# TimZaman/dotaclient

Hardware: NVIDIA H100
Metric: optimizer_steps_per_sec (higher is better)
Workload: dtype f32

## Files before the change

### dotaclient_b200/_lib.py

```python
import ctypes
import os

_HERE = os.path.dirname(os.path.abspath(__file__))
LIB_PATH = os.path.join(_HERE, "libdotaclient_b200.so")

_c = ctypes
_vp, _i32, _i64, _f32, _f64, _sz = _c.c_void_p, _c.c_int, _c.c_int64, _c.c_float, _c.c_double, _c.c_size_t
_ptr5 = _c.c_void_p * 5


class GatherDesc(_c.Structure):
    _fields_ = [("src", _vp), ("dst", _vp), ("outer", _i64), ("src_cols", _i64), ("row_bytes", _i64)]

SIGNATURES = {
    "dc_version": (_i32, []),
    "dc_last_error": (_c.c_char_p, []),
    "dc_device_info": (_i32, [_c.POINTER(_i32)] * 3),
    "dc_gae_scan": (_i32, [_vp, _i32, _vp, _vp, _i32, _vp, _vp, _f64, _f64, _vp, _vp, _vp]),
    "dc_vtrace_scan": (_i32, [_vp, _i32, _vp, _vp, _vp, _vp, _i32, _vp, _vp, _f64, _f64, _f64, _f64, _vp, _vp, _vp, _vp]),
    "dc_gae_scan_indexed": (_i32, [_vp, _i32, _vp, _i64, _vp, _vp, _i32, _vp, _vp, _f64, _f64, _vp, _vp, _vp]),
    "dc_vtrace_scan_indexed": (_i32, [_vp, _i32, _vp, _i64, _vp, _vp, _vp, _vp, _i32, _vp, _vp, _f64, _f64, _f64, _f64, _vp,
                                      _vp, _vp, _vp]),
    "dc_gather_columns": (_i32, [_c.POINTER(GatherDesc), _i32, _vp, _i64, _vp]),
    "dc_gather_columns_fill": (_i32, [_c.POINTER(GatherDesc), _i32, _vp, _i64, _vp]),
    "dc_refresh_states": (_i32, [_i32, _i32, _vp, _vp, _i64, _i64, _vp, _vp, _vp, _i64, _i64, _i64, _vp, _vp, _vp, _vp, _vp,
                                 _vp, _vp]),
    "dc_rnn_workspace_bytes": (_sz, [_i32, _i32, _i32]),
    "dc_rnn_seq_fwd": (_i32, [_i32, _vp, _vp, _vp, _vp, _vp, _i32, _i32, _i32, _vp, _vp]),
    "dc_rnn_seq_bwd": (_i32, [_i32, _vp, _vp, _vp, _vp, _vp, _vp, _vp, _vp, _vp, _i32, _i32, _i32, _vp, _vp]),
    "dc_rnn_seq_fwd_reset": (_i32, [_i32, _vp, _vp, _vp, _vp, _vp, _vp, _vp, _vp, _i32, _i32, _i32, _i32, _vp, _vp]),
    "dc_rnn_seq_bwd_reset": (_i32, [_i32, _vp, _vp, _vp, _vp, _vp, _vp, _vp, _vp, _vp, _vp, _vp, _i32, _i32, _i32, _i32, _vp,
                                    _vp]),
    "dc_gemm_tf32x3_supported": (_i32, [_i64, _i32, _i32]),
    "dc_gemm_tf32x3": (_i32, [_vp, _i32, _vp, _i32, _vp, _vp, _i32, _i64, _i32, _i32, _i32, _vp]),
    "dc_gemm_wgrad_workspace_bytes": (_sz, [_i32, _i32]),
    "dc_gemm_wgrad_tf32x3": (_i32, [_vp, _i32, _vp, _i32, _i64, _i32, _i32, _vp, _i32, _vp, _i32, _vp, _vp]),
    "dc_unit_basic_bwd_workspace_bytes": (_sz, []),
    "dc_env_fwd": (_i32, [_vp, _vp, _vp, _vp, _i32, _i64, _vp]),
    "dc_env_bwd_workspace_bytes": (_sz, []),
    "dc_env_bwd": (_i32, [_vp, _vp, _i32, _vp, _vp, _vp, _i64, _vp, _vp]),
    "dc_unit_wgrad_routed": (_i32, [_vp, _vp, _i32, _vp, _vp, _i64, _i32, _vp, _vp, _vp, _vp]),
    "dc_unit_dgrad_fused": (_i32, [_vp, _vp, _i32, _vp, _vp, _i32, _vp, _vp, _vp, _vp, _vp, _i64, _i32, _vp, _vp, _i32, _vp, _vp]),
    "dc_unit_dgrad_fused_mask": (_i32, [_vp, _vp, _i32, _vp, _vp, _i32, _vp, _vp, _vp, _vp, _vp, _vp, _i64, _i32, _vp, _vp, _i32, _vp,
                                        _vp]),
    "dc_gemm_unit_max": (_i32, [_vp, _vp, _vp, _vp, _vp, _i32, _vp, _i64, _i32, _vp]),
    "dc_unit_embed_fwd": (_i32, [_vp, _vp, _vp, _vp, _vp, _vp, _vp, _vp, _i32, _vp, _i64, _i32, _vp]),
    "dc_unit_embed_fwd_mask": (_i32, [_vp, _vp, _vp, _vp, _vp, _vp, _vp, _vp, _vp, _i32, _vp, _i64, _i32, _vp]),
    "dc_target_unit_q_fwd": (_i32, [_vp, _i32, _c.c_void_p * 6, _vp, _vp, _vp, _i64, _vp]),
    "dc_target_unit_q_bwd": (_i32, [_vp, _c.c_void_p * 6, _vp, _vp, _vp, _i32, _i64, _vp]),
    "dc_ppo_loss_fwd_bwd": (_i32, [_ptr5, _ptr5, _ptr5, _vp, _vp, _vp, _vp, _i64, _f32, _f32, _f32, _ptr5, _vp, _vp,
                                   _vp, _vp, _vp]),
    "dc_ppo_loss_fwd_bwd_strided": (_i32, [_ptr5, _c.c_int64 * 5, _ptr5, _ptr5, _vp, _vp, _vp, _vp, _i64, _i64, _f32, _f32, _f32,
                                           _ptr5, _c.c_int64 * 5, _vp, _i64, _vp, _vp, _vp, _vp]),
    "dc_ppo_loss_fwd_bwd_dev": (_i32, [_ptr5, _c.c_int64 * 5, _ptr5, _ptr5, _vp, _vp, _vp, _vp, _i64, _vp, _i64, _vp,
                                       _ptr5, _c.c_int64 * 5, _vp, _i64, _vp, _vp, _vp, _vp, _vp]),
    "dc_ppo_loss_fwd_bwd_masked": (_i32, [_ptr5, _c.c_int64 * 5, _ptr5, _ptr5, _vp, _vp, _vp, _vp, _i64, _vp, _vp, _i64,
                                          _vp, _ptr5, _c.c_int64 * 5, _vp, _i64, _vp, _vp, _vp, _vp, _vp]),
    "dc_ppo_loss_fwd_bwd_joint": (_i32, [_ptr5, _c.c_int64 * 5, _ptr5, _ptr5, _vp, _vp, _vp, _vp, _i64, _vp, _vp, _i64,
                                         _vp, _ptr5, _c.c_int64 * 5, _vp, _i64, _vp, _vp, _vp, _vp, _vp]),
    "dc_ppo_loss_fwd_bwd_kl": (_i32, [_ptr5, _c.c_int64 * 5, _ptr5, _ptr5, _vp, _vp, _vp, _vp, _vp, _i64, _vp, _vp, _i64,
                                      _vp, _i32, _ptr5, _c.c_int64 * 5, _vp, _i64, _vp, _vp, _vp, _vp, _vp, _vp]),
    "dc_selected_logp_rows": (_i32, [_ptr5, _ptr5, _ptr5, _i64, _vp, _vp, _vp]),
    "dc_value_norm_stats": (_i32, [_vp, _vp, _i64, _vp, _vp]),
    "dc_value_denorm": (_i32, [_vp, _i64, _i64, _f64, _f64, _vp, _vp]),
    "dc_value_head_rescale": (_i32, [_vp, _i64, _vp, _f64, _f64, _f64, _f64, _vp]),
    "dc_selected_logp": (_i32, [_ptr5, _ptr5, _ptr5, _i64, _vp, _vp]),
    "dc_select_actions": (_i32, [_ptr5, _c.c_int64 * 5, _ptr5, _vp, _i64, _vp, _vp, _vp]),
    "dc_grad_flags": (_i32, [_vp, _i64, _vp, _i32, _vp, _vp]),
    "dc_grad_finish": (_i32, [_vp, _vp, _vp, _vp, _vp, _vp, _vp, _vp, _i32, _i64, _f64, _f64, _f64, _f64, _f64, _vp, _vp,
                              _vp, _vp]),
    "dc_grad_finish_dev": (_i32, [_vp, _vp, _vp, _vp, _vp, _vp, _vp, _vp, _i32, _i64, _vp, _f64, _f64, _f64, _vp, _vp, _vp,
                                  _vp]),
    "dc_grad_finish_kl": (_i32, [_vp, _vp, _vp, _vp, _vp, _vp, _vp, _vp, _i32, _i64, _vp, _f64, _f64, _f64, _vp, _vp, _vp,
                                 _vp]),
}

PPO_WORKSPACE_BYTES = 512
FINISH_WORKSPACE_BYTES = 1024
LOSS_SLOTS = 16
HPARAM_SLOTS = 10
HP_LR, HP_E_CLIP, HP_ENTROPY_COEF, HP_VF_COEF, HP_MAX_GRAD_NORM, HP_VALUE_CLIP = range(6)
HP_VALUE_NORM_MEAN, HP_VALUE_NORM_STD = 6, 7
HP_KL_COEF, HP_KL_STOP = 8, 9
PPO_STATS_SLOTS = 24
STAT_APPROX_KL, STAT_CLIP_FRACTION, STAT_EXPLAINED_VAR = 0, 6, 12
STAT_JOINT_APPROX_KL, STAT_JOINT_CLIP_FRACTION = 13, 14
STAT_KL, STAT_KL_PENALTY = 16, 22
KL_ROW_FLOATS = 65
FINISH_KL_METRICS = 6
VTRACE_STATS_SLOTS = 8
GATHER_MAX_TENSORS = 32
REFRESH_MAX_LAYERS = 16
MAX_PARAM_TENSORS = 96

_lib = None


class NativeLibraryError(RuntimeError):
    pass


def load():
    global _lib
    if _lib is not None:
        return _lib
    if not os.path.exists(LIB_PATH):
        raise NativeLibraryError(
            "%s not found: build it with `python -m dotaclient_b200.build` (needs nvcc, sm_90a). "
            "dotaclient_b200 has no CPU fallback." % LIB_PATH)
    lib = ctypes.CDLL(LIB_PATH)
    for name, (res, args) in SIGNATURES.items():
        try:
            fn = getattr(lib, name)
        except AttributeError:
            continue
        fn.restype = res
        fn.argtypes = args
    _lib = lib
    return lib


def exported(name):
    lib = load()
    return hasattr(lib, name)


def check(rc, what):
    if rc != 0:
        msg = load().dc_last_error()
        raise RuntimeError("%s failed (code %d): %s" % (what, rc, msg.decode() if msg else "?"))


def ptr(t):
    return None if t is None else t.data_ptr()


def ptr5(tensors):
    return _ptr5(*[t.data_ptr() if t is not None else None for t in tensors])


def stream_ptr():
    import torch
    return torch.cuda.current_stream().cuda_stream
```

### dotaclient_b200/csrc/gemm_tf32x3.cu

```cuda
#include "dc_common.cuh"
#include "unit_basic.cuh"

namespace {

constexpr int BM = 128, BN = 128, BK = 32;
constexpr int kStages = 2;
constexpr int kTileBytes = BM * BK * 4;
constexpr int kStageBytes = 4 * kTileBytes;
constexpr int kProducerThreads = 128;
constexpr int kProducerGroups = kStages;
constexpr int kConsumerWarp0 = 4 * kProducerGroups;
constexpr int kConsumerThreads = 256;
constexpr int kThreads = kConsumerWarp0 * 32 + kConsumerThreads;
constexpr int kLdS = BN + 8;
constexpr int kDIn = kUnitFeatures;
constexpr size_t kOffStaging = (size_t)kStages * kStageBytes;
constexpr size_t kOffBars = kOffStaging + (size_t)BM * kLdS * 4;
constexpr size_t kSmemBytes = kOffBars + 128 + 1024 ;

#define DC_ACC8(b) "+f"(d[b]), "+f"(d[b + 1]), "+f"(d[b + 2]), "+f"(d[b + 3]), "+f"(d[b + 4]), "+f"(d[b + 5]), "+f"(d[b + 6]), "+f"(d[b + 7])
__device__ __forceinline__ void wgmma_m64n128k8(float (&d)[64], uint64_t desc_a, uint64_t desc_b) {
    asm volatile(
        "{\n\t.reg .pred p;\n\tsetp.ne.b32 p, %66, 0;\n\t"
        "wgmma.mma_async.sync.aligned.m64n128k8.f32.tf32.tf32 "
// ... 872 lines not shown
            const int s = j % kWgStages;
            dc_mbar_wait(&empty[s], ((j / kWgStages) & 1) ^ 1);
            unsigned char *st = ring + (size_t)s * kWgStageBytes;
            const uint32_t xs = dc_smem_u32(st + 2 * kTileBytes);
#pragma unroll
            for (int r = 0; r < BK / 4; ++r) {
                const int row = (t >> 5) + 4 * r;
                const bool ok = xc_in && t0 + row < tend;
                cp_async16(xs + (row * kWgLdX + 4 * xc) * 4, X + (ok ? (size_t)(t0 + row) * ldx + n0 + 4 * xc : 0), ok ? 16u : 0u);
            }
            cp_async_arrive(&full[s]);
            store_row_k(va, st, st + kTileBytes, t);
            asm volatile("fence.proxy.async.shared::cta;" ::: "memory");
            __syncwarp();
            if (lane == 0) dc_mbar_arrive(&full[s]);
        }
        colsum_s[g * 128 + t] = cs;
        asm volatile("cp.async.wait_all;" ::: "memory");
    } else {
        const int ct = threadIdx.x - kConsumerWarp0 * 32, wg = ct >> 7, w4 = (ct >> 5) & 3, q = lane & 3;
        const int rlo = 64 * wg + 16 * w4 + (lane >> 2);
        float d[64];
#pragma unroll
        for (int i = 0; i < 64; ++i) d[i] = 0.f;
        uint32_t ahi[2][4] = {}, alo[2][4] = {};
#pragma unroll
        for (int i = 0; i < 64; ++i) dc_reg_fence(d[i]);
        float *pt = part_w + ((size_t)split * tiles_mn + tile) * BM * BN + ct * 4;
        const auto flush = [&](bool add) {
            dc_wgmma_wait0();
#pragma unroll
            for (int k = 0; k < 64; ++k) dc_reg_fence(d[k]);
            if (add) {
#pragma unroll
                for (int m = 0; m < 16; ++m)
                    asm volatile("red.global.add.v4.f32 [%0], {%1, %2, %3, %4};" ::"l"(pt + m * kConsumerThreads * 4), "f"(d[4 * m]),
                                 "f"(d[4 * m + 1]), "f"(d[4 * m + 2]), "f"(d[4 * m + 3]) : "memory");
            } else {
#pragma unroll
                for (int m = 0; m < 16; ++m)
                    *reinterpret_cast<float4 *>(pt + m * kConsumerThreads * 4) = make_float4(d[4 * m], d[4 * m + 1], d[4 * m + 2], d[4 * m + 3]);
            }
#pragma unroll
            for (int k = 0; k < 64; ++k) d[k] = 0.f;
#pragma unroll
            for (int k = 0; k < 64; ++k) dc_reg_fence(d[k]);
        };
        int j = 0;
        do {
            const int j_end = min(my_chunks, j + kWgFlush);
            for (; j < j_end; ++j) {
                const int s = j % kWgStages;
                dc_mbar_wait(&full[s], (j / kWgStages) & 1);
                const uint32_t st = dc_smem_u32(ring + (size_t)s * kWgStageBytes);
                const uint32_t xk = st + 2 * kTileBytes + (q * kWgLdX + rlo) * 4;
                float v[16];
#pragma unroll
                for (int ks = 0; ks < BK / 8; ++ks) {
                    const uint32_t x8 = xk + 8 * ks * kWgLdX * 4;
                    v[4 * ks] = lds_f32(x8);
                    v[4 * ks + 1] = lds_f32(x8 + 8 * 4);
                    v[4 * ks + 2] = lds_f32(x8 + 4 * kWgLdX * 4);
                    v[4 * ks + 3] = lds_f32(x8 + (4 * kWgLdX + 8) * 4);
                }
                const uint64_t b_hi = dc_wgmma_desc(st), b_lo = dc_wgmma_desc(st + kTileBytes);
#pragma unroll
                for (int ks = 0; ks < BK / 8; ++ks) {
                    const int b = ks & 1;
#pragma unroll
                    for (int e = 0; e < 4; ++e) {
                        const float h = dc_tf32_rna(v[4 * ks + e]);
                        ahi[b][e] = __float_as_uint(h);
                        alo[b][e] = __float_as_uint(v[4 * ks + e] - h);
                    }
                    dc_wgmma_fence();
                    const uint64_t adv = (uint64_t)(ks * 2);
                    wgmma_m64n128k8_rs(d, ahi[b][0], ahi[b][1], ahi[b][2], ahi[b][3], b_lo + adv);
                    wgmma_m64n128k8_rs(d, alo[b][0], alo[b][1], alo[b][2], alo[b][3], b_hi + adv);
                    wgmma_m64n128k8_rs(d, ahi[b][0], ahi[b][1], ahi[b][2], ahi[b][3], b_hi + adv);
                    dc_wgmma_commit();
                    wgmma_wait1();
#pragma unroll
                    for (int e = 0; e < 4; ++e) asm volatile("" : "+r"(ahi[b ^ 1][e]), "+r"(alo[b ^ 1][e])::"memory");
                    if (ks == 0 && j > 0) {
                        __syncwarp();
                        if (lane == 0) dc_mbar_arrive(&empty[(j - 1) % kWgStages]);
                    }
                }
            }
            flush(j > kWgFlush);
        } while (j < my_chunks);
    }
    __syncthreads();
    if (part_b != nullptr && n0 == 0 && threadIdx.x < 128 && m0 + (int)threadIdx.x < No)
        part_b[(size_t)split * No + m0 + threadIdx.x] = colsum_s[threadIdx.x] + colsum_s[128 + threadIdx.x];
}

constexpr int kRedRows = 8;
__global__ void __launch_bounds__(32 * kRedRows) wgrad_reduce_kernel(const float *__restrict__ part_w, const float *__restrict__ part_b,
                                                                     int nsplit, int No, int Ni, float *__restrict__ dW, int ldw,
                                                                     float *__restrict__ db, int accumulate) {
    __shared__ float4 sh[kRedRows][32];
    const int x = threadIdx.x & 31, y = threadIdx.x >> 5;
    const int n_blocks = (Ni + BN - 1) / BN, tiles_mn = ((No + BM - 1) / BM) * n_blocks;
    const int total4 = tiles_mn * (BM * BN / 4), bias4 = db != nullptr ? No / 4 : 0;
    const int idx = blockIdx.x * 32 + x;
    const float *src = nullptr;
    size_t stride = 0;
    if (idx < total4) {
        src = part_w + (size_t)idx * 4;
        stride = (size_t)tiles_mn * BM * BN;
    } else if (idx < total4 + bias4) {
        src = part_b + (size_t)(idx - total4) * 4;
        stride = (size_t)No;
    }
    float4 acc = make_float4(0.f, 0.f, 0.f, 0.f);
    if (src != nullptr) {
#pragma unroll 4
        for (int s = y; s < nsplit; s += kRedRows) {
            const float4 v = __ldg(reinterpret_cast<const float4 *>(src + (size_t)s * stride));
            acc.x += v.x; acc.y += v.y; acc.z += v.z; acc.w += v.w;
        }
    }
    sh[y][x] = acc;
    __syncthreads();
    if (y == 0 && src != nullptr) {
        if (idx < total4) {
            const int tile = idx / (BM * BN / 4), r = idx % (BM * BN / 4), m = r / kConsumerThreads, ct = r % kConsumerThreads;
            const int o = (tile / n_blocks) * BM + 8 * m + 2 * (ct & 3);
            const int i = (tile % n_blocks) * BN + 64 * (ct >> 7) + 16 * ((ct >> 5) & 3) + ((ct & 31) >> 2);
            float *p[4];
            float v[4];
#pragma unroll
            for (int e = 0; e < 4; ++e) {
                const int oe = o + (e & 1), ie = i + 8 * (e >> 1);
                p[e] = oe < No && ie < Ni ? dW + (size_t)oe * ldw + ie : nullptr;
                v[e] = accumulate && p[e] != nullptr ? *p[e] : 0.f;
            }
#pragma unroll
            for (int r = 0; r < kRedRows; ++r) { v[0] += sh[r][x].x; v[1] += sh[r][x].y; v[2] += sh[r][x].z; v[3] += sh[r][x].w; }
#pragma unroll
            for (int e = 0; e < 4; ++e)
                if (p[e] != nullptr) *p[e] = v[e];
        } else {
            float *dst = db + (size_t)(idx - total4) * 4;
            float4 t = accumulate ? *reinterpret_cast<const float4 *>(dst) : make_float4(0.f, 0.f, 0.f, 0.f);
#pragma unroll
            for (int r = 0; r < kRedRows; ++r) { t.x += sh[r][x].x; t.y += sh[r][x].y; t.z += sh[r][x].z; t.w += sh[r][x].w; }
            *reinterpret_cast<float4 *>(dst) = t;
        }
    }
}

}

extern "C" int dc_gemm_tf32x3_supported(int64_t M, int N, int K) { return M > 0 && N > 0 && K > 0 && N % 32 == 0 && K % BK == 0; }

template <int NU, bool kGenA = false>
static int launch_ws(const float *A, int lda, const float *B, int ldb, const float *bias, float *C, int ldc, int M, int N,
                     int K, int relu, float *C_copy, uint8_t *argmax, cudaStream_t st, GenA gen = GenA{}) {
    const int tile_rows = NU == 5 ? 60 : kWsRows;
    const int n_blocks = (N + BN - 1) / BN, m_blocks = (M + tile_rows - 1) / tile_rows;
    int per_block = dc_sm_count() / n_blocks;
    if (per_block < 1) per_block = 1;
    if (per_block > m_blocks) per_block = m_blocks;
    const size_t smem = kGenA ? kWsGenSmemBytes : kWsSmemBytes;
    DC_CUDA(cudaFuncSetAttribute(gemm_ws_kernel<NU, kGenA>, cudaFuncAttributeMaxDynamicSharedMemorySize, (int)smem));
    gemm_ws_kernel<NU, kGenA><<<n_blocks * per_block, kWsThreads, smem, st>>>(A, lda, B, ldb, bias, C, ldc, M, N, K, relu, C_copy,
                                                                             argmax, gen);
    DC_LAUNCH_OK();
    return DC_OK;
}

extern "C" int dc_gemm_tf32x3(const float *A, int lda, const float *B, int ldb, const float *bias, float *C, int ldc,
                              int64_t M, int N, int K, int relu, dc_stream_t stream) {
    DC_REQUIRE(A && B && C, DC_EINVAL, "dc_gemm_tf32x3: null pointer");
    DC_REQUIRE(dc_gemm_tf32x3_supported(M, N, K) && M < (1ll << 31) - BM, DC_EUNSUPPORTED,
               "dc_gemm_tf32x3: need N %% 32 == 0 and K %% 32 == 0 (M=%lld N=%d K=%d)", (long long)M, N, K);
    DC_REQUIRE(lda >= K && ldb >= K && ldc >= N && lda % 4 == 0 && ldb % 4 == 0 && ldc % 4 == 0, DC_EINVAL,
               "dc_gemm_tf32x3: leading dimensions must be >= extent and multiples of 4 floats");
    DC_REQUIRE(((uintptr_t)A & 15) == 0 && ((uintptr_t)B & 15) == 0 && ((uintptr_t)C & 15) == 0 && (!bias || ((uintptr_t)bias & 15) == 0),
               DC_EINVAL, "dc_gemm_tf32x3: pointers must be 16-byte aligned");
    if (K <= 4 * BK) return launch_ws<0>(A, lda, B, ldb, bias, C, ldc, (int)M, N, K, relu, nullptr, nullptr, dc_cu_stream(stream));
    const int tiles = (int)((M + BM - 1) / BM) * ((N + BN - 1) / BN);
    DC_CUDA(cudaFuncSetAttribute(gemm_tf32x3_kernel, cudaFuncAttributeMaxDynamicSharedMemorySize, (int)kSmemBytes));
    const int grid = tiles < dc_sm_count() ? tiles : dc_sm_count();
    gemm_tf32x3_kernel<<<grid, kThreads, kSmemBytes, dc_cu_stream(stream)>>>(A, lda, B, ldb, bias, C, ldc, (int)M, N, K, relu, 1, 0);
    DC_LAUNCH_OK();
    return DC_OK;
}

int dc_gemm_tf32x3_splitk(const float *A, int lda, const float *B, int ldb, float *part, int64_t M, int N, int K, int ksplit,
                          bool first_call, cudaStream_t st) {
    DC_REQUIRE(A && B && part && ksplit >= 1 && N % BN == 0 && K % (BK * ksplit) == 0 && M > 0, DC_EINVAL,
               "dc_gemm_tf32x3_splitk: bad arguments (M=%lld N=%d K=%d ksplit=%d)", (long long)M, N, K, ksplit);
    if (first_call)
        DC_CUDA(cudaFuncSetAttribute(gemm_tf32x3_kernel, cudaFuncAttributeMaxDynamicSharedMemorySize, (int)kSmemBytes));
    const int tiles = (int)((M + BM - 1) / BM) * (N / BN) * ksplit;
    const int grid = tiles < dc_sm_count() ? tiles : dc_sm_count();
    gemm_tf32x3_kernel<<<grid, kThreads, kSmemBytes, st>>>(A, lda, B, ldb, nullptr, part, N, (int)M, N, K, 0, ksplit, (long long)M * N);
    DC_LAUNCH_OK();
    return DC_OK;
}

static int wgrad_tiles(int No, int Ni) { return ((No + BM - 1) / BM) * ((Ni + BN - 1) / BN); }

static int wgrad_splits(int No, int Ni) {
    const int tiles_mn = wgrad_tiles(No, Ni);
    const int n = dc_sm_count() / tiles_mn;
    return n < 1 ? 1 : n;
}

extern "C" size_t dc_gemm_wgrad_workspace_bytes(int No, int Ni) {
    if (No <= 0 || Ni <= 0 || No % 32 || Ni % 32) return 0;
    const int nsplit = wgrad_splits(No, Ni);
    return ((size_t)nsplit * wgrad_tiles(No, Ni) * BM * BN + (size_t)nsplit * No) * sizeof(float);
}

extern "C" int dc_gemm_wgrad_tf32x3(const float *dY, int ldy, const float *X, int ldx, int64_t T, int No, int Ni, float *dW,
                                    int ldw, float *db, int accumulate, void *workspace, dc_stream_t stream) {
    DC_REQUIRE(dY && X && dW && workspace, DC_EINVAL, "dc_gemm_wgrad_tf32x3: null pointer");
    DC_REQUIRE(T > 0 && T < (1ll << 31) - BK && No > 0 && Ni > 0 && No % 32 == 0 && Ni % 32 == 0, DC_EUNSUPPORTED,
               "dc_gemm_wgrad_tf32x3: need No %% 32 == 0 and Ni %% 32 == 0 (T=%lld No=%d Ni=%d)", (long long)T, No, Ni);
    DC_REQUIRE(ldy >= No && ldx >= Ni && ldw >= Ni && ldy % 4 == 0 && ldx % 4 == 0 && ldw % 4 == 0, DC_EINVAL,
               "dc_gemm_wgrad_tf32x3: bad leading dimension");
    DC_REQUIRE(((uintptr_t)dY & 15) == 0 && ((uintptr_t)X & 15) == 0 && ((uintptr_t)dW & 15) == 0 && ((uintptr_t)workspace & 15) == 0 &&
                   ((uintptr_t)db & 15) == 0,
               DC_EINVAL, "dc_gemm_wgrad_tf32x3: pointers must be 16-byte aligned");
    const int tiles_mn = wgrad_tiles(No, Ni), nsplit = wgrad_splits(No, Ni);
    float *part_w = reinterpret_cast<float *>(workspace);
    float *part_b = db ? part_w + (size_t)nsplit * tiles_mn * BM * BN : nullptr;
    cudaStream_t st = dc_cu_stream(stream);
    DC_CUDA(cudaFuncSetAttribute(gemm_wgrad_kernel<0>, cudaFuncAttributeMaxDynamicSharedMemorySize, (int)kWgSmemBytes));
    gemm_wgrad_kernel<0><<<tiles_mn * nsplit, kThreads, kWgSmemBytes, st>>>(dY, ldy, nullptr, nullptr, X, ldx, (int)T, No, Ni,
                                                                                      nsplit, part_w, part_b);
    DC_LAUNCH_OK();
    const int total4 = tiles_mn * (BM * BN / 4) + (db ? No / 4 : 0);
    wgrad_reduce_kernel<<<(total4 + 31) / 32, 32 * kRedRows, 0, st>>>(part_w, part_b, nsplit, No, Ni, dW, ldw, db, accumulate);
    DC_LAUNCH_OK();
    return DC_OK;
}

extern "C" int dc_gemm_unit_max(const float *basic, const float *w, const float *bias, float *xmax, float *xmax_copy, int ld_x,
                                uint8_t *argmax, int64_t n_tokens, int n_units, dc_stream_t stream) {
    DC_REQUIRE(basic && w && bias && xmax && argmax && n_tokens > 0, DC_EINVAL, "dc_gemm_unit_max: null pointer / empty input");
    DC_REQUIRE(n_units == 5 || n_units == 16, DC_EUNSUPPORTED, "dc_gemm_unit_max: n_units=%d (5 or 16; 1-unit groups are plain GEMMs)", n_units);
    DC_REQUIRE(ld_x >= BN && n_tokens * n_units < (1ll << 31) - BM, DC_EINVAL, "dc_gemm_unit_max: bad ld_x / size");
    DC_REQUIRE(((uintptr_t)basic & 15) == 0 && ((uintptr_t)w & 15) == 0, DC_EINVAL, "dc_gemm_unit_max: pointers must be 16-byte aligned");
    const int M = (int)(n_tokens * n_units);
    cudaStream_t st = dc_cu_stream(stream);
    if (n_units == 5) return launch_ws<5>(basic, BN, w, BN, bias, xmax, ld_x, M, BN, BN, 0, xmax_copy, argmax, st);
    return launch_ws<16>(basic, BN, w, BN, bias, xmax, ld_x, M, BN, BN, 0, xmax_copy, argmax, st);
}

extern "C" int dc_unit_embed_fwd_mask(const float *units, const float *w_b, const float *b_b, float *basic_out, uint32_t *mask_out,
                                      const float *w, const float *bias, float *xmax, float *xmax_copy, int ld_x, uint8_t *argmax,
                                      int64_t n_tokens, int n_units, dc_stream_t stream) {
    DC_REQUIRE(units && w_b && b_b && w && bias && xmax && n_tokens > 0, DC_EINVAL, "dc_unit_embed_fwd: null pointer / empty input");
    DC_REQUIRE(n_units == 1 || n_units == 5 || n_units == 16, DC_EUNSUPPORTED, "dc_unit_embed_fwd: n_units=%d (1, 5 or 16)", n_units);
    DC_REQUIRE(n_units == 1 ? (argmax == nullptr && xmax_copy == nullptr) : argmax != nullptr, DC_EINVAL,
               "dc_unit_embed_fwd: the arg-max (and the copy) go with the max-pool of n_units 5 and 16 only");
    DC_REQUIRE(ld_x >= BN && ld_x % 4 == 0 && n_tokens * n_units < (1ll << 31) - BM, DC_EINVAL, "dc_unit_embed_fwd: bad ld_x / size");
    DC_REQUIRE(((uintptr_t)units & 15) == 0 && ((uintptr_t)basic_out & 15) == 0 && ((uintptr_t)w & 15) == 0 && ((uintptr_t)bias & 15) == 0 &&
                   ((uintptr_t)xmax & 15) == 0 && ((uintptr_t)xmax_copy & 15) == 0 && ((uintptr_t)mask_out & 15) == 0,
               DC_EINVAL, "dc_unit_embed_fwd: units, basic_out, mask_out, w, bias, xmax, xmax_copy must be 16-byte aligned");
    const int M = (int)(n_tokens * n_units);
    const GenA gen{units, w_b, b_b, basic_out, mask_out};
    cudaStream_t st = dc_cu_stream(stream);
    if (n_units == 1) return launch_ws<0, true>(nullptr, BN, w, BN, bias, xmax, ld_x, M, BN, BN, 0, nullptr, nullptr, st, gen);
    if (n_units == 5) return launch_ws<5, true>(nullptr, BN, w, BN, bias, xmax, ld_x, M, BN, BN, 0, xmax_copy, argmax, st, gen);
    return launch_ws<16, true>(nullptr, BN, w, BN, bias, xmax, ld_x, M, BN, BN, 0, xmax_copy, argmax, st, gen);
}

extern "C" int dc_unit_embed_fwd(const float *units, const float *w_b, const float *b_b, float *basic_out, const float *w, const float *bias,
                                 float *xmax, float *xmax_copy, int ld_x, uint8_t *argmax, int64_t n_tokens, int n_units,
                                 dc_stream_t stream) {
    return dc_unit_embed_fwd_mask(units, w_b, b_b, basic_out, nullptr, w, bias, xmax, xmax_copy, ld_x, argmax, n_tokens, n_units, stream);
}

extern "C" int dc_unit_dgrad_fused_mask(const float *d_xmax, const float *d_xmax2, int ld_dx, const uint8_t *argmax, const float *dlogits,
                                        int ld_dl, const float *att, const float *w_t, const float *units, const uint32_t *mask,
                                        const float *w_b, const float *b_b, int64_t n_tokens, int n_units, float *dw_b, float *db_b,
                                        int accumulate, void *workspace, dc_stream_t stream) {
    DC_REQUIRE(w_t && units && w_b && b_b && dw_b && db_b && workspace && n_tokens > 0, DC_EINVAL, "dc_unit_dgrad_fused: null pointer / empty input");
    DC_REQUIRE(n_units == 1 || n_units == 5 || n_units == 16, DC_EUNSUPPORTED, "dc_unit_dgrad_fused: n_units=%d (1, 5 or 16)", n_units);
    DC_REQUIRE((d_xmax == nullptr && d_xmax2 == nullptr) || (d_xmax != nullptr && ld_dx >= BN && ld_dx % 4 == 0), DC_EINVAL,
               "dc_unit_dgrad_fused: bad d_xmax / ld_dx");
    DC_REQUIRE(d_xmax == nullptr || n_units == 1 || argmax != nullptr, DC_EINVAL, "dc_unit_dgrad_fused: routing needs the arg-max");
    DC_REQUIRE((dlogits == nullptr) == (att == nullptr) && (dlogits == nullptr || ld_dl >= n_units), DC_EINVAL,
               "dc_unit_dgrad_fused: dlogits and att come together");
    DC_REQUIRE(n_tokens * n_units < (1ll << 31) - BM, DC_EINVAL, "dc_unit_dgrad_fused: too many rows");
    DC_REQUIRE(((uintptr_t)d_xmax & 15) == 0 && ((uintptr_t)d_xmax2 & 15) == 0 && ((uintptr_t)argmax & 3) == 0 && ((uintptr_t)att & 15) == 0 &&
                   ((uintptr_t)w_t & 15) == 0 && ((uintptr_t)units & 15) == 0 && ((uintptr_t)mask & 15) == 0 && ((uintptr_t)workspace & 15) == 0,
               DC_EINVAL, "dc_unit_dgrad_fused: d_xmax, att, w_t, units, mask must be 16-byte aligned (arg-max 4-byte)");
    const int n_tok = (int)n_tokens;
    const int tile_rows = BM - BM % n_units;
    int grid = (int)((n_tokens * n_units + tile_rows - 1) / tile_rows);
    if (grid > dc_sm_count()) grid = dc_sm_count();
    float *partial = reinterpret_cast<float *>(workspace);
    cudaStream_t st = dc_cu_stream(stream);
#define DC_LAUNCH_DGRAD(NU, MASK)                                                                                                    \
    do {                                                                                                                              \
        DC_CUDA(cudaFuncSetAttribute(unit_dgrad_kernel<NU, MASK>, cudaFuncAttributeMaxDynamicSharedMemorySize, (int)kDgSmemBytes)); \
        unit_dgrad_kernel<NU, MASK><<<grid, kThreads, kDgSmemBytes, st>>>(d_xmax, d_xmax2, ld_dx, argmax, dlogits, ld_dl, att, w_t,  \
                                                                          units, mask, w_b, b_b, n_tok, partial);                     \
    } while (0)
    if (mask != nullptr) {
        if (n_units == 1) DC_LAUNCH_DGRAD(1, true);
        else if (n_units == 5) DC_LAUNCH_DGRAD(5, true);
        else DC_LAUNCH_DGRAD(16, true);
    } else {
        if (n_units == 1) DC_LAUNCH_DGRAD(1, false);
        else if (n_units == 5) DC_LAUNCH_DGRAD(5, false);
        else DC_LAUNCH_DGRAD(16, false);
    }
#undef DC_LAUNCH_DGRAD
    DC_LAUNCH_OK();
    return dc_unit_basic_reduce(partial, grid, dw_b, db_b, accumulate, st);
}

extern "C" int dc_unit_dgrad_fused(const float *d_xmax, const float *d_xmax2, int ld_dx, const uint8_t *argmax, const float *dlogits,
                                   int ld_dl, const float *att, const float *w_t, const float *units, const float *w_b,
                                   const float *b_b, int64_t n_tokens, int n_units, float *dw_b, float *db_b, int accumulate,
                                   void *workspace, dc_stream_t stream) {
    return dc_unit_dgrad_fused_mask(d_xmax, d_xmax2, ld_dx, argmax, dlogits, ld_dl, att, w_t, units, nullptr, w_b, b_b, n_tokens, n_units,
                                    dw_b, db_b, accumulate, workspace, stream);
}

extern "C" int dc_unit_wgrad_routed(const float *d_xmax, const float *d_xmax2, int ld_dx, const uint8_t *argmax, const float *basic,
                                    int64_t n_tokens, int n_units, float *dW, float *db, void *workspace, dc_stream_t stream) {
    DC_REQUIRE(d_xmax && argmax && basic && dW && db && workspace && n_tokens > 0, DC_EINVAL, "dc_unit_wgrad_routed: null pointer / empty input");
    DC_REQUIRE(n_units == 5 || n_units == 16, DC_EUNSUPPORTED, "dc_unit_wgrad_routed: n_units=%d (5 or 16; a 1-unit group is dc_gemm_wgrad_tf32x3)", n_units);
    DC_REQUIRE(ld_dx >= BM && n_tokens * n_units < (1ll << 31) - BK, DC_EINVAL, "dc_unit_wgrad_routed: bad ld_dx / size");
    DC_REQUIRE(((uintptr_t)basic & 15) == 0 && ((uintptr_t)dW & 15) == 0 && ((uintptr_t)db & 15) == 0 && ((uintptr_t)workspace & 15) == 0,
               DC_EINVAL, "dc_unit_wgrad_routed: pointers must be 16-byte aligned");
    const int No = BM, Ni = BN, nsplit = wgrad_splits(No, Ni);
// ... 19 lines not shown
```

### include/dotaclient_b200.h

```cpp
#ifndef DOTACLIENT_B200_H
#define DOTACLIENT_B200_H

#include <stddef.h>
#include <stdint.h>

#ifdef __cplusplus
extern "C" {
#endif

#define DC_OK 0
#define DC_EINVAL (-1)
#define DC_EUNSUPPORTED (-2)

#define DC_CELL_GRU 0
#define DC_CELL_LSTM 1

#define DC_NUM_HEADS 5
#define DC_LOSS_SLOTS 16

typedef void *dc_stream_t;

int dc_version(void);
const char *dc_last_error(void);
int dc_device_info(int *sm_count, int *cc_major, int *cc_minor);

int dc_gae_scan(const float *rewards, int n_sub, const float *values, const int64_t *seg_off,
                int n_seg, const float *boot_value, const float *boot_reward, double gamma,
                double lam, float *adv, float *ret, dc_stream_t stream);

#define DC_VTRACE_STATS_SLOTS 8
int dc_vtrace_scan(const float *rewards, int n_sub, const float *values, const float *logp_target,
                   const float *logp_behaviour, const int64_t *seg_off, int n_seg, const int64_t *valid_len,
                   const float *boot_value, double gamma, double lam, double rho_clip, double c_clip, float *pg_adv,
                   float *vs, double *seg_stats, dc_stream_t stream);

int dc_gae_scan_indexed(const float *rewards, int n_sub, const float *values, int64_t ld_values, const int64_t *tok,
                        const int64_t *seg_off, int n_seg, const float *boot_value, const float *boot_reward,
                        double gamma, double lam, float *adv, float *ret, dc_stream_t stream);
int dc_vtrace_scan_indexed(const float *rewards, int n_sub, const float *values, int64_t ld_values,
                           const float *logp_target, const float *logp_behaviour, const int64_t *tok,
                           const int64_t *seg_off, int n_seg, const int64_t *valid_len, const float *boot_value,
                           double gamma, double lam, double rho_clip, double c_clip, float *pg_adv, float *vs,
                           double *seg_stats, dc_stream_t stream);

typedef struct {
    const void *src;
    void *dst;
    int64_t outer;
    int64_t src_cols;
    int64_t row_bytes;
} dc_gather_desc;
#define DC_GATHER_MAX_TENSORS 32
int dc_gather_columns(const dc_gather_desc *descs, int n_desc, const int64_t *index, int64_t n_index,
                      dc_stream_t stream);
int dc_gather_columns_fill(const dc_gather_desc *descs, int n_desc, const int64_t *index, int64_t n_index,
                           dc_stream_t stream);

#define DC_REFRESH_MAX_LAYERS 16
int dc_refresh_states(int n_layers, int H, const float *const *h_bufs, const float *const *c_bufs, int64_t R, int64_t t0,
                      const int64_t *step, const int64_t *rollout, const int64_t *slot, int64_t n, int64_t B, int64_t K,
                      float *h0, float *c0, float *reset_h, float *reset_c, double *partial, double *acc,
                      dc_stream_t stream);

size_t dc_rnn_workspace_bytes(int cell, int B, int H);
int dc_rnn_seq_fwd(int cell, float *gates, const float *w_hh, const float *b_hh, float *ybuf,
                   float *cbuf, int B, int S, int H, void *workspace, dc_stream_t stream);
int dc_rnn_seq_bwd(int cell, float *gates, const float *w_hh, const float *ybuf, float *cbuf,
                   const float *dy, const float *dhn, const float *dcn, float *dh0, float *dc0,
                   int B, int S, int H, void *workspace, dc_stream_t stream);

int dc_rnn_seq_fwd_reset(int cell, float *gates, const float *w_hh, const float *b_hh, float *ybuf, float *cbuf,
                         const int32_t *reset_slot, const float *reset_prev, const float *reset_pre, int K,
                         int B, int S, int H, void *workspace, dc_stream_t stream);
int dc_rnn_seq_bwd_reset(int cell, float *gates, const float *w_hh, const float *ybuf, float *cbuf,
                         const float *dy, const float *dhn, const float *dcn, float *dh0, float *dc0,
                         const int32_t *reset_slot, const float *reset_prev, int K,
                         int B, int S, int H, void *workspace, dc_stream_t stream);

int dc_gemm_tf32x3_supported(int64_t M, int N, int K);
int dc_gemm_tf32x3(const float *A, int lda, const float *B, int ldb, const float *bias, float *C, int ldc,
                   int64_t M, int N, int K, int relu, dc_stream_t stream);

size_t dc_gemm_wgrad_workspace_bytes(int No, int Ni);
int dc_gemm_wgrad_tf32x3(const float *dY, int ldy, const float *X, int ldx, int64_t T, int No, int Ni,
                         float *dW, int ldw, float *db, int accumulate, void *workspace, dc_stream_t stream);

size_t dc_unit_basic_bwd_workspace_bytes(void);
int dc_env_fwd(const float *env, const float *w_e, const float *b_e, float *out, int ld_out, int64_t N,
               dc_stream_t stream);
size_t dc_env_bwd_workspace_bytes(void);
int dc_env_bwd(const float *d_out, const float *out, int ld, const float *env, float *dw_e, float *db_e, int64_t N,
               void *workspace, dc_stream_t stream);
int dc_gemm_unit_max(const float *basic, const float *w, const float *bias, float *xmax, float *xmax_copy, int ld_x,
                     uint8_t *argmax, int64_t n_tokens, int n_units, dc_stream_t stream);
int dc_unit_embed_fwd(const float *units, const float *w_b, const float *b_b, float *basic_out, const float *w, const float *bias,
                      float *xmax, float *xmax_copy, int ld_x, uint8_t *argmax, int64_t n_tokens, int n_units, dc_stream_t stream);
int dc_unit_embed_fwd_mask(const float *units, const float *w_b, const float *b_b, float *basic_out, uint32_t *mask_out, const float *w,
                           const float *bias, float *xmax, float *xmax_copy, int ld_x, uint8_t *argmax, int64_t n_tokens, int n_units,
                           dc_stream_t stream);
int dc_target_unit_q_fwd(const float *q, int ld_q, const float *const units[6], const float *w_b, const float *b_b, float *logits,
                         int64_t N, dc_stream_t stream);
int dc_target_unit_q_bwd(const float *dlogits, const float *const units[6], const float *w_b, const float *b_b, float *s, int ld_s,
                         int64_t N, dc_stream_t stream);
int dc_unit_wgrad_routed(const float *d_xmax, const float *d_xmax2, int ld_dx, const uint8_t *argmax, const float *basic,
                         int64_t n_tokens, int n_units, float *dW, float *db, void *workspace, dc_stream_t stream);
int dc_unit_dgrad_fused(const float *d_xmax, const float *d_xmax2, int ld_dx, const uint8_t *argmax, const float *dlogits,
                        int ld_dl, const float *att, const float *w_t, const float *units, const float *w_b,
                        const float *b_b, int64_t n_tokens, int n_units, float *dw_b, float *db_b, int accumulate,
                        void *workspace, dc_stream_t stream);
int dc_unit_dgrad_fused_mask(const float *d_xmax, const float *d_xmax2, int ld_dx, const uint8_t *argmax, const float *dlogits,
                             int ld_dl, const float *att, const float *w_t, const float *units, const uint32_t *mask, const float *w_b,
                             const float *b_b, int64_t n_tokens, int n_units, float *dw_b, float *db_b, int accumulate,
                             void *workspace, dc_stream_t stream);

#define DC_PPO_WORKSPACE_BYTES 512
int dc_ppo_loss_fwd_bwd(const float *const logits[DC_NUM_HEADS],
                        const uint8_t *const masks[DC_NUM_HEADS],
                        const uint8_t *const actions[DC_NUM_HEADS], const float *old_logp,
                        const float *adv_raw, const float *ret, const float *value, int64_t N,
                        float e_clip, float entropy_coef, float vf_coef,
                        float *const dlogits[DC_NUM_HEADS], float *dvalue, float *out,
                        int32_t *n_actions, void *workspace, dc_stream_t stream);

int dc_ppo_loss_fwd_bwd_strided(const float *const logits[DC_NUM_HEADS], const int64_t ld_logits[DC_NUM_HEADS],
                                const uint8_t *const masks[DC_NUM_HEADS],
                                const uint8_t *const actions[DC_NUM_HEADS], const float *old_logp,
                                const float *adv_raw, const float *ret, const float *value, int64_t ld_value,
                                int64_t N, float e_clip, float entropy_coef, float vf_coef,
                                float *const dlogits[DC_NUM_HEADS], const int64_t ld_dlogits[DC_NUM_HEADS],
                                float *dvalue, int64_t ld_dvalue, float *out, int32_t *n_actions,
                                void *workspace, dc_stream_t stream);

#define DC_HPARAM_SLOTS 10
#define DC_HP_LR 0
#define DC_HP_E_CLIP 1
#define DC_HP_ENTROPY_COEF 2
#define DC_HP_VF_COEF 3
#define DC_HP_MAX_GRAD_NORM 4
#define DC_HP_VALUE_CLIP 5
#define DC_HP_VALUE_NORM_MEAN 6
#define DC_HP_VALUE_NORM_STD 7
#define DC_HP_KL_COEF 8
#define DC_HP_KL_STOP 9

#define DC_PPO_STATS_SLOTS 24
#define DC_STAT_APPROX_KL 0
#define DC_STAT_CLIP_FRACTION 6
#define DC_STAT_EXPLAINED_VAR 12
#define DC_STAT_JOINT_APPROX_KL 13
#define DC_STAT_JOINT_CLIP_FRACTION 14
#define DC_STAT_KL 16
#define DC_STAT_KL_PENALTY 22
int dc_ppo_loss_fwd_bwd_dev(const float *const logits[DC_NUM_HEADS], const int64_t ld_logits[DC_NUM_HEADS],
                            const uint8_t *const masks[DC_NUM_HEADS],
                            const uint8_t *const actions[DC_NUM_HEADS], const float *old_logp,
                            const float *adv_raw, const float *ret, const float *value, int64_t ld_value,
                            const float *old_value, int64_t N, const double *hparams,
                            float *const dlogits[DC_NUM_HEADS], const int64_t ld_dlogits[DC_NUM_HEADS],
                            float *dvalue, int64_t ld_dvalue, float *out, float *stats, int32_t *n_actions,
                            void *workspace, dc_stream_t stream);

int dc_ppo_loss_fwd_bwd_masked(const float *const logits[DC_NUM_HEADS], const int64_t ld_logits[DC_NUM_HEADS],
                               const uint8_t *const masks[DC_NUM_HEADS],
                               const uint8_t *const actions[DC_NUM_HEADS], const float *old_logp,
                               const float *adv_raw, const float *ret, const float *value, int64_t ld_value,
                               const float *old_value, const uint8_t *valid, int64_t N, const double *hparams,
                               float *const dlogits[DC_NUM_HEADS], const int64_t ld_dlogits[DC_NUM_HEADS],
                               float *dvalue, int64_t ld_dvalue, float *out, float *stats, int32_t *n_actions,
                               void *workspace, dc_stream_t stream);

int dc_ppo_loss_fwd_bwd_joint(const float *const logits[DC_NUM_HEADS], const int64_t ld_logits[DC_NUM_HEADS],
                              const uint8_t *const masks[DC_NUM_HEADS],
                              const uint8_t *const actions[DC_NUM_HEADS], const float *old_logp,
                              const float *adv_raw, const float *ret, const float *value, int64_t ld_value,
                              const float *old_value, const uint8_t *valid, int64_t N, const double *hparams,
                              float *const dlogits[DC_NUM_HEADS], const int64_t ld_dlogits[DC_NUM_HEADS],
                              float *dvalue, int64_t ld_dvalue, float *out, float *stats, int32_t *n_actions,
                              void *workspace, dc_stream_t stream);

#define DC_KL_ROW_FLOATS 65
int dc_selected_logp_rows(const float *const logits[DC_NUM_HEADS], const uint8_t *const masks[DC_NUM_HEADS],
                          const uint8_t *const actions[DC_NUM_HEADS], int64_t N, float *logp_out, float *logp_rows,
                          dc_stream_t stream);
int dc_ppo_loss_fwd_bwd_kl(const float *const logits[DC_NUM_HEADS], const int64_t ld_logits[DC_NUM_HEADS],
                           const uint8_t *const masks[DC_NUM_HEADS], const uint8_t *const actions[DC_NUM_HEADS],
                           const float *old_logp, const float *old_log_probs, const float *adv_raw, const float *ret,
                           const float *value, int64_t ld_value, const float *old_value, const uint8_t *valid, int64_t N,
                           const double *hparams, int joint, float *const dlogits[DC_NUM_HEADS],
                           const int64_t ld_dlogits[DC_NUM_HEADS], float *dvalue, int64_t ld_dvalue, float *out,
                           float *stats, float *kl_out, int32_t *n_actions, void *workspace, dc_stream_t stream);

int dc_value_norm_stats(const float *x, const uint8_t *valid, int64_t N, double *out, dc_stream_t stream);
int dc_value_denorm(const float *v, int64_t ld_v, int64_t N, double mu, double sigma, float *out, dc_stream_t stream);
int dc_value_head_rescale(float *w, int64_t n, float *b, double mu_old, double sigma_old, double mu_new, double sigma_new,
                          dc_stream_t stream);

int dc_selected_logp(const float *const logits[DC_NUM_HEADS],
                     const uint8_t *const masks[DC_NUM_HEADS],
                     const uint8_t *const actions[DC_NUM_HEADS], int64_t N, float *logp_out,
                     dc_stream_t stream);

int dc_grad_flags(float *flat_grad, int64_t total, const int32_t *seg_head, int n_seg,
                  const int32_t *n_actions, dc_stream_t stream);
int dc_grad_finish(float *flat_param, float *flat_grad, float *exp_avg, float *exp_avg_sq,
                   int32_t *steps, const int64_t *seg_lo, const int64_t *seg_hi, const int32_t *seg_head, int n_seg,
                   int64_t total, double lr, double beta1, double beta2, double adam_eps,
                   double max_norm, const float *loss_out, float *metrics, void *workspace,
                   dc_stream_t stream);
int dc_grad_finish_dev(float *flat_param, float *flat_grad, float *exp_avg, float *exp_avg_sq,
                       int32_t *steps, const int64_t *seg_lo, const int64_t *seg_hi, const int32_t *seg_head, int n_seg,
                       int64_t total, const double *hparams, double beta1, double beta2, double adam_eps,
                       const float *loss_out, float *metrics, void *workspace, dc_stream_t stream);
#define DC_FINISH_WORKSPACE_BYTES 1024
#define DC_FINISH_KL_METRICS 6
int dc_grad_finish_kl(float *flat_param, float *flat_grad, float *exp_avg, float *exp_avg_sq,
                      int32_t *steps, const int64_t *seg_lo, const int64_t *seg_hi, const int32_t *seg_head, int n_seg,
                      int64_t total, const double *hparams, double beta1, double beta2, double adam_eps,
                      const float *loss_out, float *metrics, void *workspace, dc_stream_t stream);

int dc_select_actions(const float *const logits[DC_NUM_HEADS], const int64_t ld[DC_NUM_HEADS],
                      const uint8_t *const masks[DC_NUM_HEADS], const float *u, int64_t A, int32_t *chosen,
                      float *logp, dc_stream_t stream);

#ifdef __cplusplus
}
#endif
#endif
```

Baseline: 77.98.

## Add K-pipelined persistent TF32x3 GEMM kernel for K beyond four chunks

For GEMMs with K larger than four BK chunks, dc_gemm_tf32x3 now launches a new persistent kernel. It streams K chunks through a 4-stage shared-memory ring using full/empty mbarriers, with two producer groups alternating chunks and consumer warpgroups running the three-pass TF32 split wgmma. Bias and ReLU are applied in the epilogue. The previous ring kernel stays reachable as dc_gemm_tf32x3_ring. The aim is to overlap loads of A and B with tensor-core work for deep-K layers, at the cost of more complex synchronisation and different shared-memory pressure.

```diff
diff --git a/dotaclient_b200/_lib.py b/dotaclient_b200/_lib.py
--- a/dotaclient_b200/_lib.py
+++ b/dotaclient_b200/_lib.py
@@ -33,6 +33,7 @@
                                     _vp]),
     "dc_gemm_tf32x3_supported": (_i32, [_i64, _i32, _i32]),
     "dc_gemm_tf32x3": (_i32, [_vp, _i32, _vp, _i32, _vp, _vp, _i32, _i64, _i32, _i32, _i32, _vp]),
+    "dc_gemm_tf32x3_ring": (_i32, [_vp, _i32, _vp, _i32, _vp, _vp, _i32, _i64, _i32, _i32, _i32, _vp]),
     "dc_gemm_wgrad_workspace_bytes": (_sz, [_i32, _i32]),
     "dc_gemm_wgrad_tf32x3": (_i32, [_vp, _i32, _vp, _i32, _i64, _i32, _i32, _vp, _i32, _vp, _i32, _vp, _vp]),
     "dc_unit_basic_bwd_workspace_bytes": (_sz, []),
diff --git a/dotaclient_b200/csrc/gemm_tf32x3.cu b/dotaclient_b200/csrc/gemm_tf32x3.cu
--- a/dotaclient_b200/csrc/gemm_tf32x3.cu
+++ b/dotaclient_b200/csrc/gemm_tf32x3.cu
@@ -1048,6 +1048,142 @@
     }
 }
 
+constexpr int kKpStages = 4;
+constexpr int kKpStageBytes = 3 * kTileBytes;
+constexpr size_t kKpOffBars = (size_t)kKpStages * kKpStageBytes;
+constexpr size_t kKpSmemBytes = kKpOffBars + 2 * kKpStages * 8 + 1024 ;
+static_assert(kKpSmemBytes <= 227 * 1024, "pipelined K > 128 GEMM exceeds the shared-memory opt-in");
+
+__global__ void __launch_bounds__(kThreads, 1) gemm_kpipe_kernel(const float *__restrict__ A, int lda,
+                                                                 const float *__restrict__ B, int ldb,
+                                                                 const float *__restrict__ bias, float *__restrict__ C,
+                                                                 int ldc, int M, int N, int K, int relu) {
+    extern __shared__ unsigned char smem_raw[];
+    unsigned char *ring = smem_base(smem_raw);
+    uint64_t *full = reinterpret_cast<uint64_t *>(ring + kKpOffBars), *empty = full + kKpStages;
+
+    const int warp = threadIdx.x >> 5, lane = threadIdx.x & 31;
+    const int m_blocks = (M + BM - 1) / BM, n_blocks = (N + BN - 1) / BN, k_chunks = K / BK, tiles = m_blocks * n_blocks;
+    if (threadIdx.x == 0) {
+        for (int s = 0; s < kKpStages; ++s) { dc_mbar_init(&full[s], kProducerThreads + 4); dc_mbar_init(&empty[s], kConsumerThreads / 32); }
+        asm volatile("fence.mbarrier_init.release.cluster;" ::: "memory");
+    }
+    __syncthreads();
+
+    if (warp < kConsumerWarp0) {
+        const int t = threadIdx.x & (kProducerThreads - 1), g = warp >> 2, ch = t & 7;
+        uint32_t c = 0;
+        for (int tile = blockIdx.x; tile < tiles; tile += gridDim.x) {
+            const int m0 = (tile / n_blocks) * BM, n0 = (tile % n_blocks) * BN;
+            for (int kc = 0; kc < k_chunks; ++kc, ++c) {
+                if ((int)(c & 1) != g) continue;
+                float4 vb[8];
+                tile_load_k(B, ldb, n0, N, kc * BK, t, vb);
+                const int s = c % kKpStages;
+                dc_mbar_wait(&empty[s], ((c / kKpStages) & 1) ^ 1);
+                unsigned char *st = ring + (size_t)s * kKpStageBytes;
+                const uint32_t dst = dc_smem_u32(st);
+#pragma unroll
+                for (int i = 0; i < BM / 16; ++i) {
+                    const int r = (t >> 3) + 16 * i;
+                    const bool ok = m0 + r < M;
+                    cp_async16(dst + r * 128 + ((ch ^ (r & 7)) << 4), A + (ok ? (size_t)(m0 + r) * lda : 0) + kc * BK + 4 * ch, ok ? 16u : 0u);
+                }
+                cp_async_arrive(&full[s]);
+                tile_store_k(vb, st + kTileBytes, st + 2 * kTileBytes, t);
+                asm volatile("fence.proxy.async.shared::cta;" ::: "memory");
+                __syncwarp();
+                if (lane == 0) dc_mbar_arrive(&full[s]);
+            }
+        }
+        asm volatile("cp.async.wait_all;" ::: "memory");
+        return;
+    }
+
+    const int ct = threadIdx.x - kConsumerWarp0 * 32, wg = ct >> 7, w4 = (ct >> 5) & 3, q = lane & 3, g8 = lane >> 2;
+    const int rlo = 64 * wg + 16 * w4 + g8, rhi = rlo + 8;
+    const uint32_t ring_u32 = dc_smem_u32(ring);
+    float d[64];
+    uint32_t ahi[2][4] = {}, alo[2][4] = {};
+    uint32_t c = 0;
+    for (int tile = blockIdx.x; tile < tiles; tile += gridDim.x) {
+        const int m0 = (tile / n_blocks) * BM, n0 = (tile % n_blocks) * BN;
+#pragma unroll
+        for (int i = 0; i < 64; ++i) d[i] = 0.f;
+#pragma unroll
+        for (int i = 0; i < 64; ++i) dc_reg_fence(d[i]);
+        for (int kc = 0; kc < k_chunks; ++kc, ++c) {
+            const int s = c % kKpStages;
+            dc_mbar_wait(&full[s], (c / kKpStages) & 1);
+            const uint32_t st = ring_u32 + s * kKpStageBytes;
+            float v[16];
+#pragma unroll
+            for (int ks = 0; ks < BK / 8; ++ks) {
+#pragma unroll
+                for (int h = 0; h < 2; ++h) {
+                    const int j = 2 * ks + h;
+                    v[4 * ks + 2 * h] = lds_f32(st + (rlo * BK + ((j ^ (rlo & 7)) << 2) + q) * 4);
+                    v[4 * ks + 2 * h + 1] = lds_f32(st + (rhi * BK + ((j ^ (rhi & 7)) << 2) + q) * 4);
+                }
+            }
+            const uint64_t b_hi = dc_wgmma_desc(st + kTileBytes), b_lo = dc_wgmma_desc(st + 2 * kTileBytes);
+#pragma unroll
+            for (int ks = 0; ks < BK / 8; ++ks) {
+                const int b = ks & 1;
+#pragma unroll
+                for (int e = 0; e < 4; ++e) {
+                    const float h = dc_tf32_rna(v[4 * ks + e]);
+                    ahi[b][e] = __float_as_uint(h);
+                    alo[b][e] = __float_as_uint(v[4 * ks + e] - h);
+                }
+                dc_wgmma_fence();
+                const uint64_t adv = (uint64_t)(ks * 2);
+                wgmma_m64n128k8_rs(d, alo[b][0], alo[b][1], alo[b][2], alo[b][3], b_hi + adv);
+                wgmma_m64n128k8_rs(d, ahi[b][0], ahi[b][1], ahi[b][2], ahi[b][3], b_lo + adv);
+                wgmma_m64n128k8_rs(d, ahi[b][0], ahi[b][1], ahi[b][2], ahi[b][3], b_hi + adv);
+                dc_wgmma_commit();
+                wgmma_wait1();
+#pragma unroll
+                for (int e = 0; e < 4; ++e) asm volatile("" : "+r"(ahi[b ^ 1][e]), "+r"(alo[b ^ 1][e])::"memory");
+                if (ks == 0 && kc > 0) {
+                    __syncwarp();
+                    if (lane == 0) dc_mbar_arrive(&empty[(c - 1) % kKpStages]);
+                }
+            }
+        }
+        dc_wgmma_wait0();
+#pragma unroll
+        for (int e = 0; e < 4; ++e) asm volatile("" : "+r"(ahi[0][e]), "+r"(alo[0][e]), "+r"(ahi[1][e]), "+r"(alo[1][e])::"memory");
+#pragma unroll
+        for (int i = 0; i < 64; ++i) dc_reg_fence(d[i]);
+        __syncwarp();
+        if (lane == 0) dc_mbar_arrive(&empty[(c - 1) % kKpStages]);
+        const int row_lo = m0 + rlo, row_hi = m0 + rhi;
+        float *c_lo = row_lo < M ? C + (size_t)row_lo * ldc : nullptr, *c_hi = row_hi < M ? C + (size_t)row_hi * ldc : nullptr;
+        constexpr int kBiasBatch = 8;
+#pragma unroll
+        for (int g0 = 0; g0 < BN / 8; g0 += kBiasBatch) {
+            float2 bv[kBiasBatch];
+#pragma unroll
+            for (int i = 0; i < kBiasBatch; ++i) {
+                const int col = n0 + 8 * (g0 + i) + 2 * q;
+                bv[i] = bias != nullptr ? __ldg(reinterpret_cast<const float2 *>(bias + (col < N ? col : 0))) : make_float2(0.f, 0.f);
+            }
+#pragma unroll
+            for (int i = 0; i < kBiasBatch; ++i) {
+                const int g = g0 + i, col = n0 + 8 * g + 2 * q;
+                if (col >= N) break;
+                const float2 b2 = bv[i];
+                float2 lo = make_float2(d[4 * g], d[4 * g + 1]), hi = make_float2(d[4 * g + 2], d[4 * g + 3]);
+                if (bias != nullptr) { lo.x += b2.x; lo.y += b2.y; hi.x += b2.x; hi.y += b2.y; }
+                if (relu) { lo.x = fmaxf(lo.x, 0.f); lo.y = fmaxf(lo.y, 0.f); hi.x = fmaxf(hi.x, 0.f); hi.y = fmaxf(hi.y, 0.f); }
+                if (c_lo) *reinterpret_cast<float2 *>(c_lo + col) = lo;
+                if (c_hi) *reinterpret_cast<float2 *>(c_hi + col) = hi;
+            }
+        }
+    }
+}
+
 }
 
 extern "C" int dc_gemm_tf32x3_supported(int64_t M, int N, int K) { return M > 0 && N > 0 && K > 0 && N % 32 == 0 && K % BK == 0; }
@@ -1068,16 +1204,35 @@
     return DC_OK;
 }
 
+static int check_gemm_args(const char *what, const float *A, int lda, const float *B, int ldb, const float *bias, const float *C,
+                           int ldc, int64_t M, int N, int K) {
+    DC_REQUIRE(A && B && C, DC_EINVAL, "%s: null pointer", what);
+    DC_REQUIRE(dc_gemm_tf32x3_supported(M, N, K) && M < (1ll << 31) - BM, DC_EUNSUPPORTED,
+               "%s: need N %% 32 == 0 and K %% 32 == 0 (M=%lld N=%d K=%d)", what, (long long)M, N, K);
+    DC_REQUIRE(lda >= K && ldb >= K && ldc >= N && lda % 4 == 0 && ldb % 4 == 0 && ldc % 4 == 0, DC_EINVAL,
+               "%s: leading dimensions must be >= extent and multiples of 4 floats", what);
+    DC_REQUIRE(((uintptr_t)A & 15) == 0 && ((uintptr_t)B & 15) == 0 && ((uintptr_t)C & 15) == 0 && (!bias || ((uintptr_t)bias & 15) == 0),
+               DC_EINVAL, "%s: pointers must be 16-byte aligned", what);
+    return DC_OK;
+}
+
 extern "C" int dc_gemm_tf32x3(const float *A, int lda, const float *B, int ldb, const float *bias, float *C, int ldc,
                               int64_t M, int N, int K, int relu, dc_stream_t stream) {
-    DC_REQUIRE(A && B && C, DC_EINVAL, "dc_gemm_tf32x3: null pointer");
-    DC_REQUIRE(dc_gemm_tf32x3_supported(M, N, K) && M < (1ll << 31) - BM, DC_EUNSUPPORTED,
-               "dc_gemm_tf32x3: need N %% 32 == 0 and K %% 32 == 0 (M=%lld N=%d K=%d)", (long long)M, N, K);
-    DC_REQUIRE(lda >= K && ldb >= K && ldc >= N && lda % 4 == 0 && ldb % 4 == 0 && ldc % 4 == 0, DC_EINVAL,
-               "dc_gemm_tf32x3: leading dimensions must be >= extent and multiples of 4 floats");
-    DC_REQUIRE(((uintptr_t)A & 15) == 0 && ((uintptr_t)B & 15) == 0 && ((uintptr_t)C & 15) == 0 && (!bias || ((uintptr_t)bias & 15) == 0),
-               DC_EINVAL, "dc_gemm_tf32x3: pointers must be 16-byte aligned");
+    const int rc = check_gemm_args("dc_gemm_tf32x3", A, lda, B, ldb, bias, C, ldc, M, N, K);
+    if (rc != DC_OK) return rc;
     if (K <= 4 * BK) return launch_ws<0>(A, lda, B, ldb, bias, C, ldc, (int)M, N, K, relu, nullptr, nullptr, dc_cu_stream(stream));
+    const int tiles = (int)((M + BM - 1) / BM) * ((N + BN - 1) / BN);
+    DC_CUDA(cudaFuncSetAttribute(gemm_kpipe_kernel, cudaFuncAttributeMaxDynamicSharedMemorySize, (int)kKpSmemBytes));
+    const int grid = tiles < dc_sm_count() ? tiles : dc_sm_count();
+    gemm_kpipe_kernel<<<grid, kThreads, kKpSmemBytes, dc_cu_stream(stream)>>>(A, lda, B, ldb, bias, C, ldc, (int)M, N, K, relu);
+    DC_LAUNCH_OK();
+    return DC_OK;
+}
+
+extern "C" int dc_gemm_tf32x3_ring(const float *A, int lda, const float *B, int ldb, const float *bias, float *C, int ldc,
+                                   int64_t M, int N, int K, int relu, dc_stream_t stream) {
+    const int rc = check_gemm_args("dc_gemm_tf32x3_ring", A, lda, B, ldb, bias, C, ldc, M, N, K);
+    if (rc != DC_OK) return rc;
     const int tiles = (int)((M + BM - 1) / BM) * ((N + BN - 1) / BN);
     DC_CUDA(cudaFuncSetAttribute(gemm_tf32x3_kernel, cudaFuncAttributeMaxDynamicSharedMemorySize, (int)kSmemBytes));
     const int grid = tiles < dc_sm_count() ? tiles : dc_sm_count();
diff --git a/include/dotaclient_b200.h b/include/dotaclient_b200.h
--- a/include/dotaclient_b200.h
+++ b/include/dotaclient_b200.h
@@ -80,6 +80,8 @@
 int dc_gemm_tf32x3_supported(int64_t M, int N, int K);
 int dc_gemm_tf32x3(const float *A, int lda, const float *B, int ldb, const float *bias, float *C, int ldc,
                    int64_t M, int N, int K, int relu, dc_stream_t stream);
+int dc_gemm_tf32x3_ring(const float *A, int lda, const float *B, int ldb, const float *bias, float *C, int ldc,
+                        int64_t M, int N, int K, int relu, dc_stream_t stream);
 
 size_t dc_gemm_wgrad_workspace_bytes(int No, int Ni);
 int dc_gemm_wgrad_tf32x3(const float *dY, int ldy, const float *X, int ldx, int64_t T, int No, int Ni,
```

After: 79.24, median of 6. +1.6%, better.
